# mjayantkumar/spark-timeseries

Hardware: AMD Instinct MI355X
Metric: series-elements/sec + % HBM roofline (fill+lag+ACF) at 1/2/4/8 MI355X (higher is better)
Workload: dtype f64; 1 GPU; C3 shard: fill('linear') + autocorr(60), 12,500 series x 982,800 steps per GPU (N=8 -> C3's 100k x 982,800, 786 GB); series_per_gpu=12500, numLags=60, fill=linear, parallelism=dp1 (series sharded by key, one process per GPU)

## Files before the change

spark-timeseries_amd/csrc/sts_tile.hip:

```cpp
#include "sts_internal.hpp"
#include "sts_lanes.hpp"
#include "sts_acf.hpp"
#include "sts_scan.hpp"

#include <hip/hip_runtime.h>

#include <type_traits>


#ifndef STS_FILL_PRIO
#define STS_FILL_PRIO 2
#endif
#ifndef STS_TILE_WGS
#define STS_TILE_WGS 4
#endif


namespace sts {
namespace {

__device__ __forceinline__ void lds_barrier() {
    __builtin_amdgcn_fence(__ATOMIC_RELEASE, "workgroup", "local");
    __builtin_amdgcn_s_barrier();
    __builtin_amdgcn_fence(__ATOMIC_ACQUIRE, "workgroup", "local");
}

typedef double d4 __attribute__((ext_vector_type(4)));
typedef double d2v __attribute__((ext_vector_type(2)));
typedef int i4v __attribute__((ext_vector_type(4)));

constexpr int kThreads = 256;
constexpr int kBig = 1 << 30;

#ifdef STS_STAMPS
__device__ unsigned long long g_stamps[16];
#define STAMP(i)                                                                            \
    do {                                                                                    \
        const unsigned long long now_ = __builtin_amdgcn_s_memtime();                      \
        st_acc[i] += now_ - st_prev;                                                        \
        st_prev = now_;                                                                     \
    } while (0)
#else
#define STAMP(i) \
    do {         \
    } while (0)
#endif

__device__ __forceinline__ int opq(int x) {
    asm volatile("" : "+v"(x));
    return x;
}

template <int L>
__device__ __forceinline__ void wlane(int& v, unsigned x) {
    asm("v_writelane_b32 %0, %1, %2" : "+v"(v) : "s"(x), "n"(L));
}

template <int CTRL>
__device__ __forceinline__ int dpp(int old, int v) {
    return __builtin_amdgcn_update_dpp(old, v, CTRL, 0xf, 0xf, false);
}
__device__ __forceinline__ int rl(int v, int l) { return __builtin_amdgcn_readlane(v, l); }
__device__ __forceinline__ int imax(int a, int b) { return a > b ? a : b; }
__device__ __forceinline__ int imin(int a, int b) { return a < b ? a : b; }
__device__ __forceinline__ int wave_prefix_max(int v, int lane) {
    constexpr int I = -0x7fffffff - 1;
    v = imax(v, dpp<0x111>(I, v));
    v = imax(v, dpp<0x112>(I, v));
    v = imax(v, dpp<0x114>(I, v));
    v = imax(v, dpp<0x118>(I, v));
    const int p1 = rl(v, 15), p2 = imax(p1, rl(v, 31)), p3 = imax(p2, rl(v, 47));
    const int r = opq(lane) >> 4;
    return imax(v, r == 0 ? I : r == 1 ? p1 : r == 2 ? p2 : p3);
}
__device__ __forceinline__ int wave_prefix_sum(int v, int lane) {
    v += dpp<0x111>(0, v);
    v += dpp<0x112>(0, v);
    v += dpp<0x114>(0, v);
    v += dpp<0x118>(0, v);
    const int p1 = rl(v, 15), p2 = p1 + rl(v, 31), p3 = p2 + rl(v, 47);
    const int r = opq(lane) >> 4;
    return v + (r == 0 ? 0 : r == 1 ? p1 : r == 2 ? p2 : p3);
}
__device__ __forceinline__ int wave_suffix_min(int v, int lane) {
    constexpr int I = 0x7fffffff;
    v = imin(v, dpp<0x101>(I, v));
    v = imin(v, dpp<0x102>(I, v));
    v = imin(v, dpp<0x104>(I, v));
    v = imin(v, dpp<0x108>(I, v));
    const int s3 = rl(v, 48), s2 = imin(s3, rl(v, 32)), s1 = imin(s2, rl(v, 16));
    const int r = opq(lane) >> 4;
    return imin(v, r == 0 ? s1 : r == 1 ? s2 : r == 2 ? s3 : I);
}

template <bool PAD>
__device__ __forceinline__ int px_(int q) { return PAD ? q + ((q >> 5) << 2) : q; }
template <bool PAD>
__device__ __forceinline__ int px2_(int q2) { return PAD ? q2 + ((q2 >> 4) << 1) : q2; }

template <int TW, int NT, bool SHIFTED, int NTH, int M>
__global__ __launch_bounds__(NTH, STS_TILE_WGS) void tile_kernel(TileArgs a) {
    constexpr int method = M;
    if constexpr (NT > 0) __builtin_amdgcn_s_setprio(STS_FILL_PRIO);
    constexpr int kThreads = NTH;
    constexpr int kWaves = NTH / 64;
    static_assert(TW / 64 % kWaves == 0, "whole 64-step chunks per wave");
    constexpr int EW = kHB + TW + kHA;
    constexpr int NA = SHIFTED ? 2 : (NT > 0 ? NT : 1);
    constexpr int QS = (SHIFTED && NT > 0) ? 16 / NT : 16;
    constexpr int REACH = (NT == 0) ? 0 : (SHIFTED ? 80 : 16 * NT);
    constexpr bool PAD = SHIFTED && NT > 0;
    constexpr int EWP = PAD ? EW + EW / 8 : EW;
    auto px = [](int q) { return px_<PAD>(q); };
    auto px2 = [](int q2) { return px2_<PAD>(q2); };
    constexpr int PX2S = PAD ? kThreads + 2 * (kThreads / 16) : kThreads;
    constexpr int PXW = PAD ? 72 : 64;
    static_assert(kThreads % 16 == 0, "linear padded strides");
    constexpr int NW = EW / 64;
    constexpr int NP2 = EW / 2;
    constexpr int RPT = (NP2 + kThreads - 1) / kThreads;
    static_assert(EW % 64 == 0, "extended tile must be whole words");
    static_assert(NW <= 128, "word scan handles at most 128 words");
    __shared__ __attribute__((aligned(16))) double vals[EWP];
    __shared__ unsigned long long mask[NW];
    __shared__ int lastUpTo[NW];
    __shared__ int firstFrom[NW];
    constexpr int NG = NW / 8 + 1;
    constexpr int NGQ = (NG + 3) / 4;
    __shared__ __attribute__((aligned(16))) int wbase[8 * NG];
    __shared__ __attribute__((aligned(16))) int wcoarse[4 * NGQ];
    __shared__ unsigned long long wneed[NW];
    __shared__ int sh_i[4];
    __shared__ double sh_d[3];
    __shared__ int carry_L[2], carry_t[2];
    __shared__ double carry_r[2];
    __shared__ int sh_c[4];

    const int tid = threadIdx.x;
    const int lane = tid & 63;
    const int wave = __builtin_amdgcn_readfirstlane(tid >> 6);
    const int64_t nchunk = a.S * a.chunks_per_series;
    const int64_t ch = xcd_remap(blockIdx.x, nchunk);
    const int64_t s = ch / a.chunks_per_series;
    const int64_t cidx = ch - s * a.chunks_per_series;
    const int64_t k_begin = cidx * a.tiles_per_chunk;
    const int64_t k_end = (k_begin + a.tiles_per_chunk < a.tiles_per_series) ? k_begin + a.tiles_per_chunk
                                                                              : a.tiles_per_series;
    const int64_t T = a.T;
    const double* src = a.in + s * a.ld_in;
    const bool src_al = (reinterpret_cast<uintptr_t>(src) & 15) == 0;
    constexpr bool needL = (method == STS_FILL_LINEAR || method == STS_FILL_PREVIOUS || method == STS_FILL_NEAREST);
    constexpr bool needN = (method == STS_FILL_LINEAR || method == STS_FILL_NEXT || method == STS_FILL_NEAREST);
    double* dst = a.out ? a.out + s * a.ld_out : nullptr;
    const int64_t lrows = T - a.max_lag;
    const int ncols = a.max_lag + (a.include_original ? 1 : 0);
    const int init = a.include_original ? 0 : 1;

    if (tid < 2) {
        carry_L[tid] = -1;
        carry_t[tid] = -kBig;
    }
    if (tid == 0) {
        sh_c[0] = -kBig;
        sh_c[2] = -1;
    }
    if (tid < 8) {
        if (NW + 1 + tid < 8 * NG) wbase[NW + 1 + tid] = kBig;
        if (NG + tid < 4 * NGQ) wcoarse[NG + tid] = kBig;
    }
    double acc_s = 0.0, acc_q = 0.0;

    static_assert(RPT <= 9, "prefetch registers are spelled out for RPT <= 9");
    double2 R0, R1, R2, R3, R4, R5, R6, R7, R8;
    auto interior = [&](int64_t kk) {
        const int64_t e0 = kk * TW - kHB;
        return e0 >= 0 && e0 + EW <= T && src_al;
    };
#define STS_LD1(j)                                                                          \
    if constexpr (j < RPT) {                                                                \
        const int q2_ = tid + j * kThreads;                                                 \
        const double2* p_ = &s2_[q2_ < NP2 ? q2_ : NP2 - 1];                                \
        if constexpr (NT > 0) {                                                             \
            const d2v v_ = __builtin_nontemporal_load(reinterpret_cast<const d2v*>(p_));    \
            R##j = make_double2(v_.x, v_.y);                                                \
        } else {                                                                            \
            R##j = *p_;                                                                     \
        }                                                                                   \
    }
#define STS_ISSUE(kk)                                                                       \
    do {                                                                                    \
        const double2* s2_ = reinterpret_cast<const double2*>(src + ((kk) * TW - kHB));     \
        STS_LD1(0) STS_LD1(1) STS_LD1(2) STS_LD1(3) STS_LD1(4)                              \
        STS_LD1(5) STS_LD1(6) STS_LD1(7) STS_LD1(8)                                         \
    } while (0)
#define STS_CLEAR()                                                                         \
    do {                                                                                    \
        asm volatile("" : "=v"(R0), "=v"(R1), "=v"(R2), "=v"(R3), "=v"(R4));               \
        asm volatile("" : "=v"(R5), "=v"(R6), "=v"(R7), "=v"(R8));                         \
    } while (0)
#define STS_ST1(j)                                                                          \
    if constexpr (j < RPT) {                                                                \
        const int q2_ = tid + j * kThreads;                                                 \
        if ((j + 1) * kThreads <= NP2 || q2_ < NP2) v2_[pst_ + j * PX2S] = R##j;            \
    }

    d4 U[NA];
#pragma unroll
    for (int t = 0; t < NA; t++) U[t] = d4{0.0, 0.0, 0.0, 0.0};
    bool series_err = false;
#ifdef STS_STAMPS
    unsigned long long st_acc[12] = {0};
    unsigned long long st_prev = __builtin_amdgcn_s_memtime();
#endif
    bool have = interior(k_begin);
    if (have) STS_ISSUE(k_begin);
    else STS_CLEAR();
    const double c0 = [&] {
        if constexpr (NT == 0) return 0.0;
        const double v = a.shift[s];
        const unsigned long long u = __builtin_bit_cast(unsigned long long, v);
        const unsigned lo = __builtin_amdgcn_readfirstlane((unsigned)u);
        const unsigned hi = __builtin_amdgcn_readfirstlane((unsigned)(u >> 32));
        return __builtin_bit_cast(double, ((unsigned long long)hi << 32) | lo);
    }();

    constexpr int qA0 = kHB;
    constexpr int NTA = NT > 0 ? NT : 1;
    constexpr int CPW = TW / 64 / kWaves;
    auto mid_sums = [&](int p, double y) {
        const double z = acf_mid(p + lane, T) ? y : 0.0;
        acc_s += z;
        acc_q = __builtin_fma(z, z, acc_q);
    };
    auto mfma_group = [&](auto FROM, auto TO, const double* vb, int64_t kk, int tt0, int tt1) {
        constexpr int F = decltype(FROM)::value, TE = decltype(TO)::value;
        if constexpr (NT > 0 && F < TE) {
            const bool tile_mid = tt0 >= kAcfEdge && tt1 + kAcfEdge <= T;
            const int tlen = tt1 - tt0;
            const int nch = (tlen + 63) / 64;
            const bool full = wave * CPW + CPW <= nch;
            int c = wave * CPW + F;
            int cend = wave * CPW + TE;
            if (cend > nch) cend = nch;
            if constexpr (SHIFTED) {
                int oa[NTA], ob[NTA];
#pragma unroll
                for (int t = 0; t < NT; t++) {
                    const int j = lane & 15;
                    const int ra = QS * t + lane;
                    const int rb = QS * t + 16 * (lane >> 4) + 16 * (j / QS) + (16 - QS) + (j % QS);
                    oa[t] = opq(px(ra));
                    ob[t] = opq(px(rb));
                }
                auto chunk_mfma = [&](const double* yb) {
                    double av[NTA], bv[NTA];
#pragma unroll
                    for (int t = 0; t < NT; t++) {
                        av[t] = yb[oa[t]];
                        bv[t] = yb[ob[t]];
                    }
#pragma unroll
                    for (int t = 0; t < NT; t++)
                        U[t % NA] = __builtin_amdgcn_mfma_f64_16x16x4f64(av[t], bv[t], U[t % NA], 0, 0, 0);
                    return av[0];
                };
                if (F == 0 && kk == 0 && wave == 0) chunk_mfma(vb);
                if (full && tile_mid) {
                    int ia[NTA], ib[NTA];
                    const int cb = px(qA0 + 64 * (wave * CPW));
#pragma unroll
                    for (int t = 0; t < NT; t++) {
                        ia[t] = cb + oa[t];
                        ib[t] = cb + ob[t];
                        asm volatile("" : "+v"(ia[t]), "+v"(ib[t]));
                    }
#pragma unroll
                    for (int cc = F; cc < TE; cc++) {
                        double av[NTA], bv[NTA];
#pragma unroll
                        for (int t = 0; t < NT; t++) {
                            av[t] = vb[ia[t] + 72 * cc];
                            bv[t] = vb[ib[t] + 72 * cc];
                        }
#pragma unroll
                        for (int t = 0; t < NT; t++)
                            U[t % NA] = __builtin_amdgcn_mfma_f64_16x16x4f64(av[t], bv[t], U[t % NA], 0, 0, 0);
                        acc_s += av[0];
                        acc_q = __builtin_fma(av[0], av[0], acc_q);
                        __builtin_amdgcn_sched_barrier(0);
                    }
                    c = cend;
                }
                for (; c < cend; c++) mid_sums(tt0 + 64 * c, chunk_mfma(vb + px(qA0 + 64 * c)));
            } else {
                for (; c < cend; c++) {
                    const int jrel = 64 * c + lane;
                    double bv[NTA];
#pragma unroll
                    for (int t = 0; t < NT; t++) bv[t] = vb[px(qA0 + jrel + 16 * t)];
                    const double av = (jrel < tlen) ? bv[0] : 0.0;
#pragma unroll
                    for (int t = 0; t < NT; t++) U[t] = __builtin_amdgcn_mfma_f64_16x16x4f64(av, bv[t], U[t], 0, 0, 0);
                    mid_sums(tt0 + 64 * c, av);
                }
            }
        }
    };
    for (int64_t k = k_begin; k < k_end; k++) {
        const int t0 = (int)(k * TW);
        const int t1 = (t0 + TW < T) ? t0 + TW : (int)T;
        const int e0 = t0 - kHB;

        if (have) {
            double2* v2_ = reinterpret_cast<double2*>(vals);
            const int pst_ = opq(px2(tid));
            STS_ST1(0) STS_ST1(1) STS_ST1(2) STS_ST1(3) STS_ST1(4) STS_ST1(5) STS_ST1(6) STS_ST1(7) STS_ST1(8)
#define STS_BAL1(j)                                                                         \
    if constexpr (j < RPT) {                                                                \
        const unsigned long long bx_ = __ballot(!isnan_d(R##j.x));                          \
        const unsigned long long by_ = __ballot(!isnan_d(R##j.y));                          \
        const unsigned long long lo_ = interleave2((unsigned)bx_, (unsigned)by_);           \
        const unsigned long long hi_ = interleave2((unsigned)(bx_ >> 32), (unsigned)(by_ >> 32)); \
        wlane<4 * j + 0>(mv_, (unsigned)lo_);                                               \
        wlane<4 * j + 1>(mv_, (unsigned)(lo_ >> 32));                                       \
        wlane<4 * j + 2>(mv_, (unsigned)hi_);                                               \
        wlane<4 * j + 3>(mv_, (unsigned)(hi_ >> 32));                                       \
    }
            {
                int mv_ = 0;
                STS_BAL1(0) STS_BAL1(1) STS_BAL1(2) STS_BAL1(3) STS_BAL1(4) STS_BAL1(5) STS_BAL1(6)
                STS_BAL1(7) STS_BAL1(8)
                const int w_ = 2 * wave + 2 * kWaves * (lane >> 2) + ((lane >> 1) & 1);
                if (lane < 4 * RPT && w_ < NW) reinterpret_cast<int*>(mask)[2 * w_ + (lane & 1)] = mv_;
            }
#undef STS_BAL1
        } else {
            for (int q = tid; q < EW; q += kThreads) {
                const int t = e0 + q;
                vals[px(q)] = (t >= 0 && t < T) ? src[t] : __builtin_nan("");
            }
        }
        const bool have_next = (k + 1 < k_end) && interior(k + 1);
        STAMP(0);
        lds_barrier();
        STAMP(1);

        const int qA = kHB;
        const int qW = kHB + (t1 - t0);
        int qB = qW + REACH;
        if (e0 + qB > T) qB = (int)T - e0;

        if (!have) {
            const int pb = opq(px(lane) + PXW * wave);
#pragma unroll 1
            for (int i = 0; i < (NW + kWaves - 1) / kWaves; i++) {
                const int w = wave + i * kWaves;
                if (w < NW) {
                    const unsigned long long m = __ballot(!isnan_d(vals[pb + PXW * kWaves * i]));
                    if (lane == 0) mask[w] = m;
                }
            }
            STAMP(2);
            lds_barrier();
        }
        STAMP(3);

        if (wave == 0) {
            if constexpr (NT > 0) __builtin_amdgcn_s_setprio(3);
            int w0 = 2 * lane;
            asm volatile("" : "+v"(w0));
            const int w1 = w0 + 1;
            const unsigned long long m0 = (w0 < NW) ? mask[w0] : ~0ull;
            const unsigned long long m1 = (w1 < NW) ? mask[w1] : ~0ull;
            const int l0 = (w0 < NW && m0) ? w0 * 64 + 63 - __clzll(m0) : -1;
            const int l1 = (w1 < NW && m1) ? w1 * 64 + 63 - __clzll(m1) : -1;
            const int f0 = (w0 < NW && m0) ? w0 * 64 + __ffsll(m0) - 1 : kBig;
            const int f1 = (w1 < NW && m1) ? w1 * 64 + __ffsll(m1) - 1 : kBig;
            auto need = [&](int w, unsigned long long m) -> unsigned long long {
                const int lo = qA - w * 64, hi = qB - w * 64;
                if (method == STS_FILL_NONE || hi <= 0 || lo >= 64) return 0ull;
                unsigned long long r = ~m;
                if (lo > 0) r &= ~0ull << lo;
                if (hi < 64) r &= (1ull << hi) - 1ull;
                return r;
            };
            const unsigned long long n0 = (w0 < NW) ? need(w0, m0) : 0ull;
            const unsigned long long n1 = (w1 < NW) ? need(w1, m1) : 0ull;
            const int pm = wave_prefix_max(l1 > l0 ? l1 : l0, lane);
            const int sm = wave_suffix_min(f0 < f1 ? f0 : f1, lane);
            const int pc = wave_prefix_sum(__popcll(n0) + __popcll(n1), lane);
            const int ex = dpp<0x138>(-1, pm);
            const int exc = dpp<0x138>(0, pc);
            const int exs = dpp<0x130>(kBig, sm);
            const int nnan = rl(pc, 63);
            const int firstValidE = rl(sm, 0);
            const int lastValidE = rl(pm, 63);
            const bool lg = method == STS_FILL_LINEAR &&
                            __ballot((w0 < NW && __popcll(~m0) > kLongRun / 2) ||
                                     (w1 < NW && __popcll(~m1) > kLongRun / 2)) != 0ull;
            if (w0 < NW) {
                lastUpTo[w0] = ex > l0 ? ex : l0;
                const int a0 = f1 < exs ? f1 : exs;
                firstFrom[w0] = f0 < a0 ? f0 : a0;
                wbase[w0] = exc;
                wneed[w0] = n0;
                if ((lane & 3) == 0) wcoarse[lane >> 2] = exc;
            }
            if (w1 < NW) {
                const int a1 = ex > l0 ? ex : l0;
                lastUpTo[w1] = a1 > l1 ? a1 : l1;
                firstFrom[w1] = f1 < exs ? f1 : exs;
                wbase[w1] = exc + __popcll(n0);
                wneed[w1] = n1;
            }
            int lext = -1, next = (int)T;
            if (needL && e0 > 0 && firstValidE > qA && nnan > 0)
                lext = (sh_c[0] == e0) ? sh_c[1] : (int)scan_back(src, e0, lane);
            if (needN && e0 + EW < T && qB > qA && lastValidE < qB - 1 && nnan > 0) {
                const int from = e0 + EW;
                const int cN_pos = sh_c[2], cN = sh_c[3];
                next = (cN_pos >= 0 && cN_pos <= from && cN >= from) ? cN : (int)scan_fwd(src, from, T, lane);
                if (lane == 0) {
                    sh_c[2] = from;
                    sh_c[3] = next;
                }
            }
            if (needL) {
                const int lq = rl(pm, TW / 128 - 1);
                if (lane == 0) {
                    sh_c[0] = e0 + TW;
                    sh_c[1] = (lq >= 0) ? e0 + lq : lext;
                }
            }
            if (lane == 0) {
                wbase[NW] = nnan;
                if constexpr (NW % 8 == 0) wcoarse[NW / 8] = nnan;
                sh_i[0] = lext;
                sh_i[1] = next;
                sh_i[2] = nnan;
                sh_i[3] = lg ? 1 : 0;
            }
            if (lext >= 0) {
                const double v = src[lext];
                if (lane == 0) sh_d[1] = v;
            }
            if (next < T) {
                const double v = src[next];
                if (lane == 0) sh_d[2] = v;
            }
        }
        if constexpr (NT > 0) __builtin_amdgcn_s_setprio(STS_FILL_PRIO);
        STAMP(4);
        lds_barrier();
        STAMP(5);

        {
            const int nnan = sh_i[2];
            const int lext = sh_i[0], next = sh_i[1];
            const double lextv = sh_d[1], nextv = sh_d[2];
            auto impute = [&](auto long_tag) {
            constexpr bool LONG = decltype(long_tag)::value;
            for (int idx = tid; idx < nnan; idx += kThreads) {
                const i4v* c4 = reinterpret_cast<const i4v*>(wcoarse);
                int g = -1;
#pragma unroll
                for (int j = 0; j < NGQ; j++) {
                    const i4v c = c4[j];
                    g += (c.x <= idx) + (c.y <= idx) + (c.z <= idx) + (c.w <= idx);
                }
                const i4v* b4 = reinterpret_cast<const i4v*>(wbase) + 2 * g;
                const i4v ba = b4[0], bb = b4[1];
                const int w = 8 * g - 1 + (ba.x <= idx) + (ba.y <= idx) + (ba.z <= idx) + (ba.w <= idx) +
                              (bb.x <= idx) + (bb.y <= idx) + (bb.z <= idx) + (bb.w <= idx);
                unsigned long long nm = wneed[w];
                const int wb = wbase[w];
                const unsigned long long m = mask[w];
                const int lup = needL ? lastUpTo[w > 0 ? w - 1 : 0] : -1;
                const int ffr = needN ? firstFrom[w + 1 < NW ? w + 1 : NW - 1] : kBig;
                int kk = idx - wb, b = 0;
#pragma unroll
                for (int width = 32; width >= 1; width >>= 1) {
                    const int c = __popcll(nm & ((1ull << width) - 1ull));
                    if (kk >= c) { kk -= c; nm >>= width; b += width; }
                }
                const int q = w * 64 + b;
                const int t = e0 + q;
                int Lt = -1, Nt = (int)T;
                double Lv = 0.0, Nv = 0.0;
                if (needL) {
                    const unsigned long long lo = m & ((1ull << b) - 1ull);
                    const int Lq = lo ? w * 64 + 63 - __clzll(lo) : (w > 0 ? lup : -1);
                    if (Lq >= 0) { Lt = e0 + Lq; Lv = vals[px(Lq)]; }
                    else { Lt = lext; Lv = lextv; }
                }
                if (needN) {
                    const unsigned long long hi = (b == 63) ? 0ull : (m & (~0ull << (b + 1)));
                    const int Nq = hi ? w * 64 + __ffsll(hi) - 1 : (w + 1 < NW ? ffr : kBig);
                    if (Nq < kBig) { Nt = e0 + Nq; Nv = vals[px(Nq)]; }
                    else { Nt = next; Nv = nextv; }
                }
                double f = __builtin_nan("");
                switch (method) {
                case STS_FILL_PREVIOUS:
                    if (Lt >= 0) f = Lv;
                    break;
                case STS_FILL_NEXT:
                    if (Nt < T) f = Nv;
                    break;
                case STS_FILL_NEAREST: {
                    if (t == 0) break;
                    const int P = (Lt >= 1) ? Lt : -1;
                    if (P < 0 && Nt >= T) { series_err = true; break; }
                    f = (Nt >= T || (P >= 0 && t - P < Nt - t)) ? Lv : Nv;
                    break;
                }
                case STS_FILL_LINEAR: {
                    if (Lt < 0 || Nt >= T) break;
                    if (LONG && t - Lt > kLongRun) {
                        if (t - Lt == kLongRun + 1 || q == qA) {
                            const double inc = (Nv - Lv) / (double)(Nt - Lt);
                            const int rd = (int)((k + 1) & 1), wr = (int)(k & 1);
                            double v;
                            if (carry_L[rd] == Lt && carry_t[rd] == t - 1) {
                                v = carry_r[rd];
                            } else {
                                v = Lv;
                                int j = t - 1 - Lt;
                                for (; j >= 8; j -= 8) {
                                    v = v + inc; v = v + inc; v = v + inc; v = v + inc;
                                    v = v + inc; v = v + inc; v = v + inc; v = v + inc;
                                }
                                for (; j > 0; j--) v = v + inc;
                            }
                            const int qend = (Nt - e0 < qB) ? Nt - e0 : qB;
                            for (int qq = q; qq < qend; qq++) {
                                v = v + inc;
                                vals[px(qq)] = v;
                                if (e0 + qq == t1 - 1) {
                                    carry_L[wr] = Lt;
                                    carry_t[wr] = t1 - 1;
                                    carry_r[wr] = v;
                                }
                            }
                        }
                        continue;
                    }
                    const double inc = (Nv - Lv) / (double)(Nt - Lt);
                    double r = Lv;
                    for (int j = t - Lt; j > 0; j--) r = r + inc;
                    f = r;
                    break;
                }
                default:
                    break;
                }
                vals[px(q)] = f;
            }
        };
            if (sh_i[3]) impute(std::true_type{});
            else impute(std::false_type{});
        }
        STAMP(6);
        lds_barrier();
        STAMP(7);

        {
            const bool al = dst && ((reinterpret_cast<uintptr_t>(dst) & 15) == 0);
            double2* v2 = reinterpret_cast<double2*>(vals);
            const int qBfull = (NT > 0) ? ((SHIFTED || qW + 64 + 16 * NT >= EW) ? EW : qW + 64 + 16 * NT) : 0;
            const bool fast = (dst == nullptr || al) && (t1 - t0 == TW) && (NT == 0 || e0 + qW + REACH <= T);
            if (fast) {
                constexpr int FS = TW / 2 / kThreads;
                constexpr int FY = NT > 0 ? (NP2 - kHB / 2 + kThreads - 1) / kThreads : FS;
                constexpr int FH = (FY + 1) / 2;
                const int vq = (kHB >> 1) + tid;
                const int pvq = opq(px2(vq));
                const bool wr = dst != nullptr;
                char* const dpb = reinterpret_cast<char*>(dst + t0);
                unsigned dpo = (unsigned)tid * 16u;
                asm volatile("" : "+v"(dpo));
#pragma unroll
                for (int h = 0; h < 2; h++) {
                    double2 fv[FH];
#pragma unroll
                    for (int j = 0; j < FH; j++) {
                        const int jj = h * FH + j;
                        if (jj < FY && (jj * kThreads + kThreads <= NP2 - kHB / 2 ||
                                        tid + jj * kThreads < NP2 - kHB / 2))
                            fv[j] = v2[pvq + jj * PX2S];
                    }
#pragma unroll
                    for (int j = 0; j < FH; j++) {
                        const int jj = h * FH + j;
                        if (jj >= FY) continue;
                        const bool in = jj * kThreads + kThreads <= NP2 - kHB / 2 ||
                                        tid + jj * kThreads < NP2 - kHB / 2;
                        if (jj < FS && wr) {
                            double2* dq = reinterpret_cast<double2*>(dpb + jj * kThreads * 16 + dpo);
                            __builtin_nontemporal_store(fv[j].x, &dq->x);
                            __builtin_nontemporal_store(fv[j].y, &dq->y);
                        }
                        if (NT > 0 && in) {
                            double2 y;
                            y.x = fv[j].x - c0;
                            y.y = fv[j].y - c0;
                            v2[pvq + jj * PX2S] = y;
                        }
                    }
                }
            } else
            for (int q2 = (qA >> 1) + tid; 2 * q2 < qW || 2 * q2 < qBfull; q2 += kThreads) {
                const int q = 2 * q2;
                double2 f = v2[px2(q2)];
                if (q < qW) {
                    const int t = e0 + q;
                    if (dst) {
                        if (al && q + 1 < qW) {
                            *reinterpret_cast<double2*>(dst + t) = f;
                        } else {
                            dst[t] = f.x;
                            if (q + 1 < qW) dst[t + 1] = f.y;
                        }
                    }
                }
                if (NT > 0 && q < qBfull) {
                    f.x = (q < qB) ? f.x - c0 : 0.0;
                    f.y = (q + 1 < qB) ? f.y - c0 : 0.0;
                    v2[px2(q2)] = f;
                }
            }
            if (SHIFTED && NT > 0 && e0 < 0 && tid < kHB / 2) v2[px2(tid)] = make_double2(0.0, 0.0);
        }
        if (have_next) STS_ISSUE(k + 1);
        else STS_CLEAR();
        if constexpr (NT == 0) {
            if (a.lagmat) {
                double* lm = a.lagmat + s * lrows * ncols;
                for (int c = init; c <= a.max_lag; c++) {
                    double* col = lm + (int64_t)(c - init) * lrows;
                    const int sh = a.max_lag - c;
                    const int rlo = t0 - sh > 0 ? t0 - sh : 0;
                    const int rhi = (int64_t)(t1 - sh) < lrows ? t1 - sh : (int)lrows;
                    if (rlo >= rhi) continue;
                    const int par = (int)((reinterpret_cast<uintptr_t>(col) >> 3) & 1);
                    const int rp = rlo - ((rlo + par) & 1);
                    for (int r = rp + 2 * tid; r < rhi; r += 2 * kThreads) {
                        const int q = r + sh - e0;
                        if (r >= rlo && r + 1 < rhi) {
                            *reinterpret_cast<d2v*>(col + r) = d2v{vals[px(q)], vals[px(q + 1)]};
                        } else {
                            if (r >= rlo) col[r] = vals[px(q)];
                            if (r + 1 < rhi) col[r + 1] = vals[px(q + 1)];
                        }
                    }
                }
            }
        }
        STAMP(8);

        if constexpr (NT > 0) {
            lds_barrier();
            STAMP(9);
            __builtin_amdgcn_s_setprio(0);
            mfma_group(std::integral_constant<int, 0>{}, std::integral_constant<int, CPW>{}, vals, k, t0, t1);
            __builtin_amdgcn_s_setprio(STS_FILL_PRIO);
        }
        have = have_next;
        STAMP(10);
        lds_barrier();
        STAMP(11);
    }
#undef STS_ISSUE
#undef STS_LD1
#undef STS_ST1
#undef STS_CLEAR
    if (series_err && a.err) a.err[s] = STS_ERR_ALL_NAN;
#ifdef STS_STAMPS
    if (lane == 0) {
#pragma unroll
        for (int i = 0; i < 12; i++) atomicAdd(&g_stamps[i], st_acc[i]);
        atomicAdd(&g_stamps[12], 1ull);
    }
#endif

    if constexpr (NT > 0) {
        double* scr = vals + wave * 256;
        double lagacc = 0.0;
        if constexpr (SHIFTED) {
            d4 D = U[0];
#pragma unroll
            for (int t = 1; t < NA; t++) D += U[t];
#pragma unroll
            for (int r = 0; r < 4; r++) scr[((lane >> 4) + 4 * r) * 16 + (lane & 15)] = D[r];
            lds_barrier();
#pragma unroll
            for (int j = 0; j < 16; j++) {
                const int i = 16 * (j / QS) + (16 - QS) + (j % QS) - lane;
                if (i >= 0 && i < 16) lagacc += scr[i * 16 + j];
            }
            lds_barrier();
        } else {
#pragma unroll
            for (int t = 0; t < NT; t++) {
#pragma unroll
                for (int r = 0; r < 4; r++) scr[((lane >> 4) + 4 * r) * 16 + (lane & 15)] = U[t][r];
                lds_barrier();
#pragma unroll
                for (int b = 0; b < 16; b++)
                    if (((b + lane) >> 4) == t) lagacc += scr[b * 16 + ((b + lane) & 15)];
                lds_barrier();
            }
        }
#pragma unroll
        for (int d = 32; d >= 1; d >>= 1) {
            acc_s += __shfl_xor(acc_s, d);
            acc_q += __shfl_xor(acc_q, d);
        }
        double* wsum = vals + kWaves * 256;
        wsum[wave * kPartStride + lane] = lagacc;
        if (lane == 0) {
            wsum[wave * kPartStride + kPartSum] = acc_s;
            wsum[wave * kPartStride + kPartSq] = acc_q;
        }
        lds_barrier();
        if (wave == 0) {
            double* part = a.partials + ch * kPartStride;
            double tot = 0.0;
#pragma unroll
            for (int w = 0; w < kWaves; w++) tot += wsum[w * kPartStride + lane];
            part[lane] = tot;
            if (lane == 0) {
                double ts = 0.0, tq = 0.0;
#pragma unroll
                for (int w = 0; w < kWaves; w++) {
                    ts += wsum[w * kPartStride + kPartSum];
                    tq += wsum[w * kPartStride + kPartSq];
                }
                part[kPartSum] = ts;
                part[kPartSq] = tq;
                part[kPartShift] = c0;
            }
        }
    }
}

__global__ __launch_bounds__(256) void acf_finalize_kernel(FinalizeArgs a) {
    const int lane = threadIdx.x & 63;
    const int64_t s = (int64_t)blockIdx.x * 4 + (threadIdx.x >> 6);
    if (s >= a.S) return;
    const int K = a.K;
    const int i = lane + 1;
    const int64_t T = a.T;
    const double* F = a.F + s * a.ldF;
    if (lane >= K) return;
    double out;
    if (i >= T) {
        out = __builtin_nan("");
    } else if (T <= 2 * (int64_t)K || T < 2 * kAcfEdge) {
        out = acf_exact_lag(F, T, i);
    } else {
        double Pi = 0.0, Sm = 0.0, Qm = 0.0;
        const double* pp = a.partials + s * a.parts_per_series * kPartStride;
        const double c = pp[kPartShift];
        for (int64_t k = 0; k < a.parts_per_series; k++, pp += kPartStride) {
            Pi += pp[i];
            Sm += pp[kPartSum];
            Qm += pp[kPartSq];
        }
        bool sus;
        out = acf_combine(Pi, Sm, Qm, i, T, [&](int j) { return F[j] - c; },
                          [&](int j) { return F[T - 1 - j] - c; }, c, &sus);
        if (__ballot(sus) && lane == 0) a.exact[s] = 1;
    }
    a.acf[s * K + lane] = out;
}

constexpr int kExactChunk = 512;
template <bool WIDE>
__global__ __launch_bounds__(256) void acf_exact_kernel(const double* __restrict__ F, int64_t S, int64_t T,
                                                        int64_t ld, int K, int nblk, const int32_t* __restrict__ flags,
                                                        double* __restrict__ acf) {
    __shared__ double lds[4][kExactChunk + 64];
    __shared__ double ldsb[4][WIDE ? kExactChunk : 1];
    const int wave = threadIdx.x >> 6, lane = threadIdx.x & 63;
    const int nb = WIDE ? nblk - 1 : 1;
    const int64_t u = (int64_t)blockIdx.x * 4 + wave;
    const int64_t s = u / nb;
    if (s >= S || !flags[s]) return;
    const int b = WIDE ? 1 + (int)(u % nb) : 0;
    const int i = b * 64 + lane + 1;
    const bool active = i <= K && (int64_t)i < T;
    const double r = WIDE ? acf_exact_stream<kExactChunk, true>(F + s * ld, T, i, active, lds[wave], lane, b * 64,
                                                                ldsb[wave])
                          : acf_exact_stream<kExactChunk>(F + s * ld, T, i, active, lds[wave], lane);
    if (active) acf[s * K + (i - 1)] = r;
}

__global__ __launch_bounds__(256) void acf_shift_kernel(const double* in, int64_t S, int64_t T, int64_t ld, int prev,
                                                        double* shift) {
    const int lane = threadIdx.x & 63;
    const int64_t s = (int64_t)blockIdx.x * 4 + (threadIdx.x >> 6);
    if (s >= S) return;
    const double c = robust_shift(in + s * ld, T, lane, prev != 0);
    if (lane == 0) shift[s] = c;
}

}

hipError_t launch_acf_shift(const double* in, int64_t S, int64_t T, int64_t ld, int method, double* shift,
                            hipStream_t st) {
    if (S <= 0 || T <= 0) return hipSuccess;
    dim3 grid((unsigned)((S + 3) / 4)), block(256);
    hipLaunchKernelGGL(acf_shift_kernel, grid, block, 0, st, in, S, T, ld, method == STS_FILL_PREVIOUS ? 1 : 0,
                       shift);
    return hipGetLastError();
}

template <int TW, int NT, bool SHIFTED, int NTH>
hipError_t launch_m(int method, dim3 grid, const TileArgs& a, hipStream_t st) {
    const dim3 block(NTH);
    switch (method) {
    case STS_FILL_NONE: hipLaunchKernelGGL((tile_kernel<TW, NT, SHIFTED, NTH, STS_FILL_NONE>), grid, block, 0, st, a); break;
    case STS_FILL_LINEAR: hipLaunchKernelGGL((tile_kernel<TW, NT, SHIFTED, NTH, STS_FILL_LINEAR>), grid, block, 0, st, a); break;
    case STS_FILL_NEAREST: hipLaunchKernelGGL((tile_kernel<TW, NT, SHIFTED, NTH, STS_FILL_NEAREST>), grid, block, 0, st, a); break;
    case STS_FILL_NEXT: hipLaunchKernelGGL((tile_kernel<TW, NT, SHIFTED, NTH, STS_FILL_NEXT>), grid, block, 0, st, a); break;
    case STS_FILL_PREVIOUS: hipLaunchKernelGGL((tile_kernel<TW, NT, SHIFTED, NTH, STS_FILL_PREVIOUS>), grid, block, 0, st, a); break;
    default: return hipErrorInvalidValue;
    }
    return hipGetLastError();
}

hipError_t launch_tile(int method, int tw, const TileArgs& a, hipStream_t st) {
    const int64_t nchunk = a.S * a.chunks_per_series;
    if (nchunk <= 0) return hipSuccess;
    if (nchunk > 0x7fffffffLL) return hipErrorInvalidValue;
    dim3 grid((unsigned)nchunk);
    if (tw == 512 && a.K == 0) return launch_m<512, 0, false, kThreads>(method, grid, a, st);
#ifdef STS_AB
    if (tw == 2048 && a.K > 0 && a.K <= 60) {
        if (a.K <= 24) return launch_m<2048, 2, true, kThreads / 2>(method, grid, a, st);
        return launch_m<2048, 4, true, kThreads / 2>(method, grid, a, st);
    }
#endif
    if (tw != 4096) return hipErrorInvalidValue;
    if (a.K == 0) return launch_m<4096, 0, false, kThreads>(method, grid, a, st);
    if (a.K <= 24) return launch_m<4096, 2, true, kThreads>(method, grid, a, st);
    if (a.K <= 60) return launch_m<4096, 4, true, kThreads>(method, grid, a, st);
    if (a.K <= 63) return launch_m<4096, 5, false, kThreads>(method, grid, a, st);
    return hipErrorInvalidValue;
}

#ifdef STS_STAMPS
extern "C" int sts_debug_stamps(unsigned long long* out16) {
    if (hipMemcpyFromSymbol(out16, HIP_SYMBOL(g_stamps), sizeof(unsigned long long) * 16) != hipSuccess) return 4;
    unsigned long long z[16] = {0};
    return hipMemcpyToSymbol(HIP_SYMBOL(g_stamps), z, sizeof(z)) == hipSuccess ? 0 : 4;
}
#endif

hipError_t launch_acf_finalize(const FinalizeArgs& a, hipStream_t st) {
    if (a.S <= 0 || a.K <= 0) return hipSuccess;
    dim3 grid((unsigned)((a.S + 3) / 4)), block(256);
    hipLaunchKernelGGL(acf_finalize_kernel, grid, block, 0, st, a);
    return hipGetLastError();
}

hipError_t launch_acf_exact(const double* F, int64_t S, int64_t T, int64_t ldF, int K, const int32_t* exact,
                            double* acf, hipStream_t st) {
    if (S <= 0 || K <= 0 || T <= 0) return hipSuccess;
    const int nblk = (K + 63) / 64;
    if ((S * nblk + 3) / 4 > 0x7fffffffLL) return hipErrorInvalidValue;
    hipLaunchKernelGGL(acf_exact_kernel<false>, dim3((unsigned)((S + 3) / 4)), dim3(256), 0, st, F, S, T, ldF, K, nblk,
                       exact, acf);
    hipError_t e = hipGetLastError();
    if (e != hipSuccess || nblk == 1) return e;
    hipLaunchKernelGGL(acf_exact_kernel<true>, dim3((unsigned)((S * (nblk - 1) + 3) / 4)), dim3(256), 0, st, F, S, T,
                       ldF, K, nblk, exact, acf);
    return hipGetLastError();
}

}
```

Baseline: 298.6 billion series-elements/s.

## Specialize interior tiles to drop edge tests and use SGPR-based addressing

Splits the per-series tile loop into a head tile, a run of interior tiles compiled with a constant flag, and a tail, so interior tiles skip boundary clamps, end tests and the scalar-edge paths in fill and MFMA. Interior loads and stores use scalar base pointers plus fixed per-thread offsets in the global address space, and the copy-out uses nontemporal stores. Lambdas are forced inline. This targets instruction and VGPR overhead in the hot loop, at the cost of larger code and more register pressure from the duplicated tile body.

```diff
diff --git a/spark-timeseries_amd/csrc/sts_tile.hip b/spark-timeseries_amd/csrc/sts_tile.hip
--- a/spark-timeseries_amd/csrc/sts_tile.hip
+++ b/spark-timeseries_amd/csrc/sts_tile.hip
@@ -28,6 +28,8 @@
 typedef double d4 __attribute__((ext_vector_type(4)));
 typedef double d2v __attribute__((ext_vector_type(2)));
 typedef int i4v __attribute__((ext_vector_type(4)));
+typedef __attribute__((address_space(1))) char gchar;
+typedef __attribute__((address_space(1))) d2v gd2v;
 
 constexpr int kThreads = 256;
 constexpr int kBig = 1 << 30;
@@ -172,7 +174,7 @@
 
     static_assert(RPT <= 9, "prefetch registers are spelled out for RPT <= 9");
     double2 R0, R1, R2, R3, R4, R5, R6, R7, R8;
-    auto interior = [&](int64_t kk) {
+    auto interior = [&](int64_t kk) __attribute__((always_inline)) {
         const int64_t e0 = kk * TW - kHB;
         return e0 >= 0 && e0 + EW <= T && src_al;
     };
@@ -192,6 +194,33 @@
         const double2* s2_ = reinterpret_cast<const double2*>(src + ((kk) * TW - kHB));     \
         STS_LD1(0) STS_LD1(1) STS_LD1(2) STS_LD1(3) STS_LD1(4)                              \
         STS_LD1(5) STS_LD1(6) STS_LD1(7) STS_LD1(8)                                         \
+    } while (0)
+#define STS_LDIN(j)                                                                         \
+    if constexpr (j < RPT) {                                                                \
+        const unsigned o_ = ((j + 1) * kThreads <= NP2) ? ((j & 1) ? lo2_ : lo_) : lc_;     \
+        const gd2v* p_ = (const gd2v*)(lb_[j / 2] + o_);                                    \
+        if constexpr (NT > 0) {                                                             \
+            const d2v v_ = __builtin_nontemporal_load(p_);                                  \
+            R##j = make_double2(v_.x, v_.y);                                                \
+        } else {                                                                            \
+            const d2v v_ = *p_;                                                             \
+            R##j = make_double2(v_.x, v_.y);                                                \
+        }                                                                                   \
+    }
+#define STS_ISSUE_IN(kk)                                                                    \
+    do {                                                                                    \
+        constexpr int LSTR_ = kThreads * 16;                                                \
+        const int tc_ = (NP2 - 1) - (RPT - 1) * kThreads;    \
+        unsigned lo_ = (unsigned)tid * 16u, lo2_ = (unsigned)tid * 16u + LSTR_;             \
+        unsigned lc_ = (unsigned)(tid < tc_ ? tid : tc_) * 16u + ((RPT - 1) & 1) * LSTR_;   \
+        asm volatile("" : "+v"(lo_), "+v"(lo2_), "+v"(lc_));                                \
+        const gchar* lb_[(RPT + 1) / 2];                                                    \
+        _Pragma("unroll") for (int m_ = 0; m_ < (RPT + 1) / 2; m_++) {                      \
+            lb_[m_] = (const gchar*)(src + ((kk) * TW - kHB)) + 2 * m_ * LSTR_;             \
+            asm volatile("" : "+s"(lb_[m_]));                                               \
+        }                                                                                   \
+        STS_LDIN(0) STS_LDIN(1) STS_LDIN(2) STS_LDIN(3) STS_LDIN(4)                         \
+        STS_LDIN(5) STS_LDIN(6) STS_LDIN(7) STS_LDIN(8)                                     \
     } while (0)
 #define STS_CLEAR()                                                                         \
     do {                                                                                    \
@@ -227,18 +256,20 @@
     constexpr int qA0 = kHB;
     constexpr int NTA = NT > 0 ? NT : 1;
     constexpr int CPW = TW / 64 / kWaves;
-    auto mid_sums = [&](int p, double y) {
+    auto mid_sums = [&](int p, double y) __attribute__((always_inline)) {
         const double z = acf_mid(p + lane, T) ? y : 0.0;
         acc_s += z;
         acc_q = __builtin_fma(z, z, acc_q);
     };
-    auto mfma_group = [&](auto FROM, auto TO, const double* vb, int64_t kk, int tt0, int tt1) {
+    auto mfma_group = [&](auto itag, auto FROM, auto TO, const double* vb, int64_t kk, int tt0, int tt1)
+                          __attribute__((always_inline)) {
+        constexpr bool IN = decltype(itag)::value;
         constexpr int F = decltype(FROM)::value, TE = decltype(TO)::value;
         if constexpr (NT > 0 && F < TE) {
-            const bool tile_mid = tt0 >= kAcfEdge && tt1 + kAcfEdge <= T;
+            const bool tile_mid = IN || (tt0 >= kAcfEdge && tt1 + kAcfEdge <= T);
             const int tlen = tt1 - tt0;
             const int nch = (tlen + 63) / 64;
-            const bool full = wave * CPW + CPW <= nch;
+            const bool full = IN || wave * CPW + CPW <= nch;
             int c = wave * CPW + F;
             int cend = wave * CPW + TE;
             if (cend > nch) cend = nch;
@@ -252,7 +283,7 @@
                     oa[t] = opq(px(ra));
                     ob[t] = opq(px(rb));
                 }
-                auto chunk_mfma = [&](const double* yb) {
+                auto chunk_mfma = [&](const double* yb) __attribute__((always_inline)) {
                     double av[NTA], bv[NTA];
 #pragma unroll
                     for (int t = 0; t < NT; t++) {
@@ -264,7 +295,8 @@
                         U[t % NA] = __builtin_amdgcn_mfma_f64_16x16x4f64(av[t], bv[t], U[t % NA], 0, 0, 0);
                     return av[0];
                 };
-                if (F == 0 && kk == 0 && wave == 0) chunk_mfma(vb);
+                if constexpr (!IN)
+                    if (F == 0 && kk == 0 && wave == 0) chunk_mfma(vb);
                 if (full && tile_mid) {
                     int ia[NTA], ib[NTA];
                     const int cb = px(qA0 + 64 * (wave * CPW));
@@ -291,7 +323,8 @@
                     }
                     c = cend;
                 }
-                for (; c < cend; c++) mid_sums(tt0 + 64 * c, chunk_mfma(vb + px(qA0 + 64 * c)));
+                if constexpr (!IN)
+                    for (; c < cend; c++) mid_sums(tt0 + 64 * c, chunk_mfma(vb + px(qA0 + 64 * c)));
             } else {
                 for (; c < cend; c++) {
                     const int jrel = 64 * c + lane;
@@ -306,10 +339,13 @@
             }
         }
     };
-    for (int64_t k = k_begin; k < k_end; k++) {
+    static_assert(REACH <= kHA && kAcfEdge <= kHB && kAcfEdge <= kHA, "an interior tile needs no end test");
+    auto tile = [&](int64_t k, auto itag, bool have, bool want_next) __attribute__((always_inline)) -> bool {
+        constexpr bool IN = decltype(itag)::value;
         const int t0 = (int)(k * TW);
-        const int t1 = (t0 + TW < T) ? t0 + TW : (int)T;
+        const int t1 = (IN || t0 + TW < T) ? t0 + TW : (int)T;
         const int e0 = t0 - kHB;
+        if constexpr (IN) have = true;
 
         if (have) {
             double2* v2_ = reinterpret_cast<double2*>(vals);
@@ -340,7 +376,7 @@
                 vals[px(q)] = (t >= 0 && t < T) ? src[t] : __builtin_nan("");
             }
         }
-        const bool have_next = (k + 1 < k_end) && interior(k + 1);
+        const bool have_next = IN ? want_next : (k + 1 < k_end) && interior(k + 1);
         STAMP(0);
         lds_barrier();
         STAMP(1);
@@ -348,7 +384,7 @@
         const int qA = kHB;
         const int qW = kHB + (t1 - t0);
         int qB = qW + REACH;
-        if (e0 + qB > T) qB = (int)T - e0;
+        if (!IN && e0 + qB > T) qB = (int)T - e0;
 
         if (!have) {
             const int pb = opq(px(lane) + PXW * wave);
@@ -376,7 +412,7 @@
             const int l1 = (w1 < NW && m1) ? w1 * 64 + 63 - __clzll(m1) : -1;
             const int f0 = (w0 < NW && m0) ? w0 * 64 + __ffsll(m0) - 1 : kBig;
             const int f1 = (w1 < NW && m1) ? w1 * 64 + __ffsll(m1) - 1 : kBig;
-            auto need = [&](int w, unsigned long long m) -> unsigned long long {
+            auto need = [&](int w, unsigned long long m) __attribute__((always_inline)) -> unsigned long long {
                 const int lo = qA - w * 64, hi = qB - w * 64;
                 if (method == STS_FILL_NONE || hi <= 0 || lo >= 64) return 0ull;
                 unsigned long long r = ~m;
@@ -414,7 +450,7 @@
                 wneed[w1] = n1;
             }
             int lext = -1, next = (int)T;
-            if (needL && e0 > 0 && firstValidE > qA && nnan > 0)
+            if (needL && (IN || e0 > 0) && firstValidE > qA && nnan > 0)
                 lext = (sh_c[0] == e0) ? sh_c[1] : (int)scan_back(src, e0, lane);
             if (needN && e0 + EW < T && qB > qA && lastValidE < qB - 1 && nnan > 0) {
                 const int from = e0 + EW;
@@ -458,7 +494,7 @@
             const int nnan = sh_i[2];
             const int lext = sh_i[0], next = sh_i[1];
             const double lextv = sh_d[1], nextv = sh_d[2];
-            auto impute = [&](auto long_tag) {
+            auto impute = [&](auto long_tag) __attribute__((always_inline)) {
             constexpr bool LONG = decltype(long_tag)::value;
             for (int idx = tid; idx < nnan; idx += kThreads) {
                 const i4v* c4 = reinterpret_cast<const i4v*>(wcoarse);
@@ -569,7 +605,58 @@
             double2* v2 = reinterpret_cast<double2*>(vals);
             const int qBfull = (NT > 0) ? ((SHIFTED || qW + 64 + 16 * NT >= EW) ? EW : qW + 64 + 16 * NT) : 0;
             const bool fast = (dst == nullptr || al) && (t1 - t0 == TW) && (NT == 0 || e0 + qW + REACH <= T);
-            if (fast) {
+            if constexpr (IN) {
+                auto pass = [&](auto wtag) __attribute__((always_inline)) {
+                    constexpr bool WR = decltype(wtag)::value;
+                    constexpr int FS = TW / 2 / kThreads;
+                    constexpr int FY = NT > 0 ? (NP2 - kHB / 2 + kThreads - 1) / kThreads : FS;
+                    constexpr int FH = (FY + 1) / 2;
+                    constexpr int SSTR = kThreads * 16;
+                    const int pvq = opq(px2((kHB >> 1) + tid));
+                    unsigned dpo = (unsigned)tid * 16u;
+                    unsigned dpo2 = (unsigned)tid * 16u + SSTR;
+                    asm volatile("" : "+v"(dpo), "+v"(dpo2));
+                    constexpr int VL = NP2 - kHB / 2 - (FY - 1) * kThreads;
+                    const int pvl = opq(px2((kHB >> 1) + (tid < VL ? tid : VL - 1)));
+                    gchar* sb[(FS + 1) / 2];
+                    if constexpr (WR) {
+#pragma unroll
+                        for (int m = 0; m < (FS + 1) / 2; m++) {
+                            sb[m] = (gchar*)(dst + t0) + 2 * m * SSTR;
+                            asm volatile("" : "+s"(sb[m]));
+                        }
+                    }
+#pragma unroll
+                    for (int h = 0; h < 2; h++) {
+                        double2 fv[FH];
+#pragma unroll
+                        for (int j = 0; j < FH; j++) {
+                            const int jj = h * FH + j;
+                            if (jj < FY) fv[j] = v2[(jj * kThreads + kThreads <= NP2 - kHB / 2 ? pvq : pvl) + jj * PX2S];
+                        }
+#pragma unroll
+                        for (int j = 0; j < FH; j++) {
+                            const int jj = h * FH + j;
+                            if (jj >= FY) continue;
+                            if constexpr (WR) {
+                                if (jj < FS) {
+                                    gchar* dq = sb[jj / 2] + ((jj & 1) ? dpo2 : dpo);
+                                    __builtin_nontemporal_store(d2v{fv[j].x, fv[j].y}, (gd2v*)dq);
+                                }
+                            }
+                            if (NT > 0 && (jj * kThreads + kThreads <= NP2 - kHB / 2 ||
+                                           tid + jj * kThreads < NP2 - kHB / 2)) {
+                                double2 y;
+                                y.x = fv[j].x - c0;
+                                y.y = fv[j].y - c0;
+                                v2[pvq + jj * PX2S] = y;
+                            }
+                        }
+                    }
+                };
+                if (dst != nullptr) pass(std::true_type{});
+                else pass(std::false_type{});
+            } else if (fast) {
                 constexpr int FS = TW / 2 / kThreads;
                 constexpr int FY = NT > 0 ? (NP2 - kHB / 2 + kThreads - 1) / kThreads : FS;
                 constexpr int FH = (FY + 1) / 2;
@@ -629,10 +716,14 @@
                     v2[px2(q2)] = f;
                 }
             }
-            if (SHIFTED && NT > 0 && e0 < 0 && tid < kHB / 2) v2[px2(tid)] = make_double2(0.0, 0.0);
-        }
-        if (have_next) STS_ISSUE(k + 1);
-        else STS_CLEAR();
+            if (!IN && SHIFTED && NT > 0 && e0 < 0 && tid < kHB / 2) v2[px2(tid)] = make_double2(0.0, 0.0);
+        }
+        if (have_next) {
+            if constexpr (IN) STS_ISSUE_IN(k + 1);
+            else STS_ISSUE(k + 1);
+        } else {
+            STS_CLEAR();
+        }
         if constexpr (NT == 0) {
             if (a.lagmat) {
                 double* lm = a.lagmat + s * lrows * ncols;
@@ -662,16 +753,35 @@
             lds_barrier();
             STAMP(9);
             __builtin_amdgcn_s_setprio(0);
-            mfma_group(std::integral_constant<int, 0>{}, std::integral_constant<int, CPW>{}, vals, k, t0, t1);
+            mfma_group(itag, std::integral_constant<int, 0>{}, std::integral_constant<int, CPW>{}, vals, k, t0, t1);
             __builtin_amdgcn_s_setprio(STS_FILL_PRIO);
         }
-        have = have_next;
         STAMP(10);
         lds_barrier();
         STAMP(11);
-    }
+        return have_next;
+    };
+    const int kb = (int)k_begin, ke = (int)k_end;
+    int ki0 = kb, ki1 = kb;
+    if (src_al && (dst == nullptr || (reinterpret_cast<uintptr_t>(dst) & 15) == 0)) {
+        ki0 = kb > 0 ? kb : 1;
+        ki1 = ke > ki0 ? ke : ki0;
+        while (ki1 > ki0 && !interior(ki1 - 1)) ki1--;
+    }
+    int k = kb;
+    if (k < ki0) have = tile(k++, std::false_type{}, have, false);
+    if (k < ki1) {
+        do {
+            tile(k, std::true_type{}, true, k + 1 < ki1);
+            k++;
+        } while (k < ki1);
+        have = false;
+    }
+    for (; k < ke; k++) have = tile(k, std::false_type{}, have, false);
 #undef STS_ISSUE
 #undef STS_LD1
+#undef STS_ISSUE_IN
+#undef STS_LDIN
 #undef STS_ST1
 #undef STS_CLEAR
     if (series_err && a.err) a.err[s] = STS_ERR_ALL_NAN;
```

Measured after the change: 307.3 billion series-elements/s, median of 6. 2.9% higher.
